# pierotofy/OpenSplat

Hardware: NVIDIA H100
Metric: fwd_bwd_mpixel_per_s (higher is better)
Workload: dtype f32

## Files before the change

### opensplat_b200/csrc/raster_bwd.cu

```cuda
#include "raster_common.cuh"

int gsb_blend_grid(const void *kernel, int num_tiles);

namespace {

__device__ __forceinline__ float rcp_approx(float x) {
    float y;
    asm("rcp.approx.ftz.f32 %0, %1;" : "=f"(y) : "f"(x));
    return y;
}

__device__ __forceinline__ void zero_row(float *grad_rows, int k) {
    float4 *row = reinterpret_cast<float4 *>(grad_rows + (size_t)k * GSB_GRAD_ROW_FLOATS);
    const float4 z = make_float4(0.f, 0.f, 0.f, 0.f);
    row[0] = z; row[1] = z; row[2] = z;
}

constexpr int BWD_MIN_BLOCKS = 6;
template <bool SAT>
__global__ void __launch_bounds__(RK_THREADS, BWD_MIN_BLOCKS)
rasterize_backward_kernel(int img_h, int img_w, int tiles_x, int num_tiles,
                          const int2 *__restrict__ tile_bins, const GsbRecord *__restrict__ records,
                          const float *__restrict__ background, const float *__restrict__ final_Ts,
                          const int *__restrict__ final_idx, const float *__restrict__ v_output,
                          const float *__restrict__ v_output_alpha, float *__restrict__ grad_rows,
                          unsigned *__restrict__ tile_counter, const int *__restrict__ tile_order) {
    __shared__ WarpRing rings[RK_WARPS];
    const int warp = threadIdx.x >> 5, lane = threadIdx.x & 31;
    WarpRing &ring = rings[warp];
    if (lane == 0) {
#pragma unroll
        for (int s = 0; s < RK_STAGES; ++s) mbar_init(&ring.full[s], 1);
        mbar_fence_init();
    }
    __syncwarp();
    const float bg0 = __ldg(background), bg1 = __ldg(background + 1), bg2 = __ldg(background + 2);
    unsigned gchunk = 0;

    while (true) {
        int tile = 0;
        if (lane == 0) tile = (int)atomicAdd(tile_counter, 1u);
        tile = __shfl_sync(0xffffffffu, tile, 0);
        if (tile >= num_tiles) break;
        if (tile_order) tile = __ldg(tile_order + tile);
        const int2 range = tile_bins[tile];
        if (range.y <= range.x) continue;

        const int tx = tile % tiles_x, ty = tile / tiles_x;
        const int X = tx * GSB_TILE + (lane & 15);
        const int Y0 = ty * GSB_TILE + (lane >> 4);
        const float px = (float)X;
        const float tile_x0 = (float)(tx * GSB_TILE), tile_y0 = (float)(ty * GSB_TILE);

        float T[RK_PIX], Bq[RK_PIX];
        const float py0 = (float)Y0;
        float vor[RK_PIX], vog[RK_PIX], vob[RK_PIX];
        int binf[RK_PIX];
        int my_max = -1;
#pragma unroll
        for (int j = 0; j < RK_PIX; ++j) {
            const int Y = Y0 + 2 * j;
            if (X < img_w && Y < img_h) {
                const size_t p = (size_t)Y * img_w + X;
                const float Tf = final_Ts[p];
                T[j] = Tf;
                vor[j] = v_output[3 * p]; vog[j] = v_output[3 * p + 1]; vob[j] = v_output[3 * p + 2];
                binf[j] = final_idx[p];
                if (SAT) {
                    const int f = binf[j];
                    if (f & GSB_SAT_BIT0) vor[j] = 0.f;
                    if (f & (GSB_SAT_BIT0 << 1)) vog[j] = 0.f;
                    if (f & (GSB_SAT_BIT0 << 2)) vob[j] = 0.f;
                    binf[j] = f & ~GSB_SAT_MASK;
                }
                const float voa = v_output_alpha ? v_output_alpha[p] : 0.f;
                Bq[j] = -(Tf * (voa - (bg0 * vor[j] + bg1 * vog[j] + bg2 * vob[j])));
            } else {
                T[j] = 1.f; vor[j] = vog[j] = vob[j] = 0.f; Bq[j] = 0.f;
                binf[j] = -1;
            }
            my_max = max(my_max, binf[j]);
        }
        const int warp_max = __reduce_max_sync(0xffffffffu, my_max);
        const int hi = min(range.y - 1, max(warp_max, range.x - 1));

        for (int idx = hi + 1 + lane; idx < range.y; idx += 32)
            zero_row(grad_rows, __float_as_int(__ldg(&records[idx].q0.w)));
        const int L = hi - range.x + 1;
        if (L <= 0) continue;
        const int nchunks = (L + RK_CHUNK - 1) / RK_CHUNK;

        const unsigned g0 = gchunk;
        auto stage_of = [&](int c) { return (g0 + (unsigned)c) % RK_STAGES; };
        auto parity_of = [&](int c) { return ((g0 + (unsigned)c) / RK_STAGES) & 1u; };
        auto chunk_lo = [&](int c) { return max(range.x, hi + 1 - (c + 1) * RK_CHUNK); };
        auto chunk_cnt = [&](int c) { return (hi + 1 - c * RK_CHUNK) - chunk_lo(c); };
        auto issue = [&](int c) {
            if (lane == 0) {
                const unsigned s = stage_of(c);
                const uint32_t bytes = (uint32_t)chunk_cnt(c) * (uint32_t)sizeof(GsbRecord);
                mbar_arrive_expect_tx(&ring.full[s], bytes);
                tma_load_1d(&ring.rec[s][0], records + chunk_lo(c), bytes, &ring.full[s]);
            }
        };
        const int pro = min(RK_STAGES, nchunks);
        for (int c = 0; c < pro; ++c) issue(c);
        int issued = pro;

        for (int c = 0; c < nchunks; ++c) {
            const unsigned s = stage_of(c);
            mbar_wait(&ring.full[s], parity_of(c));
            const int lo = chunk_lo(c), cnt = chunk_cnt(c);
            unsigned my_mask = 0;
            if (lane < cnt) {
                my_mask = record_slot_mask(ring.rec[s][lane], tile_x0, tile_y0);
                if (my_mask == 0u) zero_row(grad_rows, __float_as_int(ring.rec[s][lane].q0.w));
            }
            unsigned live = __ballot_sync(0xffffffffu, my_mask != 0u);
            while (live) {
                const int t = 31 - __clz(live);
                live &= ~(1u << t);
                const unsigned rm = __shfl_sync(0xffffffffu, my_mask, t);
                const int idx = lo + t;
                const float4 q0 = ring.rec[s][t].q0;
                const float4 q1 = ring.rec[s][t].q1;
                const float4 q2 = ring.rec[s][t].q2;
                const float smax = fmaxf(0.f, fmaf(q0.z, GSB_LN2, GSB_SMAX_BIAS));
                const float dx = q0.x - px;
                const float adx2 = q1.x * dx * dx;
                const float bdx = q1.y * dx;
                const float dy0 = q0.y - py0;
                float s0 = 0.f, s1 = 0.f, s2 = 0.f;
                float a_r = 0.f, a_g = 0.f, a_b = 0.f;
                bool any = false;
                const int jlo = __ffs(rm) - 1, jhi = 31 - __clz(rm);
#define GSB_BWD_SLOT(j)                                                                                   \
    {                                                                                                     \
        const float dy = dy0 - (float)(2 * j);                                                                      \
        const float sigma = fmaf(dy, fmaf(q1.z, dy, bdx), adx2);                                          \
        if (__float_as_uint(sigma) <= __float_as_uint(smax)) {                    \
            const float au = ex2_approx(fmaf(sigma, -GSB_LOG2E, q0.z));           \
            const float alpha = fminf(0.99f, au);                                                         \
            if (idx <= binf[j] && alpha >= (1.f / 255.f)) {                                               \
                any = true;                                                                               \
                const float ra = rcp_approx(1.f - alpha);                                                 \
                T[j] *= ra;                                                                               \
                const float fac = alpha * T[j];                                                           \
                a_r = fmaf(fac, vor[j], a_r);                                                             \
                a_g = fmaf(fac, vog[j], a_g);                                                             \
                a_b = fmaf(fac, vob[j], a_b);                                                             \
                const float d = fmaf(q2.z, vob[j], fmaf(q2.y, vog[j], q2.x * vor[j]));   \
                const float v_alpha = fmaf(d, T[j], -(ra * Bq[j]));                                       \
                Bq[j] = fmaf(d, fac, Bq[j]);                                                              \
                 \
                const float w = au * v_alpha;                                                             \
                const float wdy = w * dy;                                                                 \
                s0 += w;                                                                                  \
                s1 += wdy;                                                                                \
                s2 = fmaf(wdy, dy, s2);                                                                   \
            }                                                                                             \
        }                                                                                                 \
        if (jhi == j) break;                                                                              \
    }
                switch (jlo) {
                    case 0: GSB_BWD_SLOT(0)
                    case 1: GSB_BWD_SLOT(1)
                    case 2: GSB_BWD_SLOT(2)
                    case 3: GSB_BWD_SLOT(3)
                    case 4: GSB_BWD_SLOT(4)
                    case 5: GSB_BWD_SLOT(5)
                    case 6: GSB_BWD_SLOT(6)
                    default: GSB_BWD_SLOT(7)
                }
#undef GSB_BWD_SLOT
                const int k = __float_as_int(q0.w);
                float *row = grad_rows + (size_t)k * GSB_GRAD_ROW_FLOATS;
                if (!__any_sync(0xffffffffu, any)) {
                    if (lane < 9) row[lane] = 0.f;
                    continue;
                }
                const float sx = dx * s0;
                float v0 = s0, v1 = sx, v2 = s1, v3 = dx * sx, v4 = dx * s1, v5 = s2, v6 = a_r, v7 = a_g;
                float v8 = a_b;
                {
                    const bool up = lane & 16;
                    const float t0 = up ? v0 : v4, t1 = up ? v1 : v5, t2 = up ? v2 : v6, t3 = up ? v3 : v7;
                    const float k0 = up ? v4 : v0, k1 = up ? v5 : v1, k2 = up ? v6 : v2, k3 = up ? v7 : v3;
                    v0 = k0 + __shfl_xor_sync(0xffffffffu, t0, 16);
                    v1 = k1 + __shfl_xor_sync(0xffffffffu, t1, 16);
                    v2 = k2 + __shfl_xor_sync(0xffffffffu, t2, 16);
                    v3 = k3 + __shfl_xor_sync(0xffffffffu, t3, 16);
                }
                {
                    const bool up = lane & 8;
                    const float t0 = up ? v0 : v2, t1 = up ? v1 : v3;
                    const float k0 = up ? v2 : v0, k1 = up ? v3 : v1;
                    v0 = k0 + __shfl_xor_sync(0xffffffffu, t0, 8);
                    v1 = k1 + __shfl_xor_sync(0xffffffffu, t1, 8);
                }
                {
                    const bool up = lane & 4;
                    const float t0 = up ? v0 : v1;
                    const float k0 = up ? v1 : v0;
                    v0 = k0 + __shfl_xor_sync(0xffffffffu, t0, 4);
                }
                v0 += __shfl_xor_sync(0xffffffffu, v0, 2);
                v0 += __shfl_xor_sync(0xffffffffu, v0, 1);
#pragma unroll
                for (int o = 16; o > 0; o >>= 1) v8 += __shfl_xor_sync(0xffffffffu, v8, o);
                const bool w8 = (lane == 1);
                if (((lane & 3) == 0) || w8) row[w8 ? 8 : (lane >> 2)] = w8 ? v8 : v0;
            }
            __syncwarp();
            if (issued < nchunks) { issue(issued); ++issued; }
        }
        gchunk = g0 + (unsigned)issued;
        __syncwarp();
    }
}

__global__ void __launch_bounds__(256)
reduce_grad_rows_kernel(int n, const int *__restrict__ cum_tiles_hit, const float *__restrict__ grad_rows,
                        const float *__restrict__ conics, const float *__restrict__ opacities,
                        float2 *__restrict__ v_xy, float *__restrict__ v_conic,
                        float *__restrict__ v_colors, float *__restrict__ v_opacity) {
    const int g = blockIdx.x * blockDim.x + threadIdx.x;
    if (g >= n) return;
    const int k0 = g ? cum_tiles_hit[g - 1] : 0, k1 = cum_tiles_hit[g];
    float a[9] = {0.f, 0.f, 0.f, 0.f, 0.f, 0.f, 0.f, 0.f, 0.f};
    for (int k = k0; k < k1; ++k) {
        const float4 *row = reinterpret_cast<const float4 *>(grad_rows + (size_t)k * GSB_GRAD_ROW_FLOATS);
        const float4 r0 = row[0], r1 = row[1];
        const float r8 = reinterpret_cast<const float *>(row)[8];
        a[0] += r0.x; a[1] += r0.y; a[2] += r0.z; a[3] += r0.w;
        a[4] += r1.x; a[5] += r1.y; a[6] += r1.z; a[7] += r1.w;
        a[8] += r8;
    }
    const float S0 = a[0], Sx = a[1], Sy = a[2], Sxx = a[3], Sxy = a[4], Syy = a[5];
    const float ca = conics[3 * g], cb = conics[3 * g + 1], cc = conics[3 * g + 2];
    const float op = opacities[g];
    v_xy[g] = make_float2(-(ca * Sx + cb * Sy), -(cb * Sx + cc * Sy));
    v_conic[3 * g] = -0.5f * Sxx; v_conic[3 * g + 1] = -0.5f * Sxy; v_conic[3 * g + 2] = -0.5f * Syy;
    v_colors[3 * g] = a[6]; v_colors[3 * g + 1] = a[7]; v_colors[3 * g + 2] = a[8];
    v_opacity[g] = (op > 0.f) ? S0 / op : 0.f;
}

}

extern "C" size_t gsb_raster_grad_rows_bytes(int m) {
    return gsb_align_up((size_t)(m > 0 ? m : 0) * GSB_GRAD_ROW_FLOATS * 4 + 256, 256);
}

extern "C" int gsb_rasterize_backward(int img_h, int img_w, int tiles_x, int tiles_y, int n, int m,
                                      const int32_t *tile_bins, const int32_t *tile_order, const float *conics,
                                      const float *opacities, void *records, const int32_t *cum_tiles_hit,
                                      const float *background, const float *final_Ts, const int32_t *final_idx,
                                      const float *v_output, const float *v_output_alpha, void *grad_rows,
                                      float *v_xy, float *v_conic, float *v_colors, float *v_opacity, unsigned flags,
                                      gsb_stream_t stream) {
    GSB_CHECK_ARG(img_h > 0 && img_w > 0 && n >= 0 && m >= 0);
    GSB_CHECK_ARG((flags & ~(unsigned)GSB_RASTER_CLAMP_MAX_ONE) == 0);
    const bool sat = (flags & GSB_RASTER_CLAMP_MAX_ONE) != 0;
    GSB_CHECK_ARG(tiles_x == gsb_div_up(img_w, GSB_TILE) && tiles_y == gsb_div_up(img_h, GSB_TILE));
    if (n == 0) return 0;
    GSB_CHECK_ARG(tile_bins && conics && opacities && cum_tiles_hit && background && final_Ts && final_idx &&
                  v_output && v_xy && v_conic && v_colors && v_opacity);
    GSB_CHECK_ARG(((uintptr_t)v_xy % 8) == 0);
    cudaStream_t s = (cudaStream_t)stream;
    if (m > 0) {
        GSB_CHECK_ARG(records && grad_rows && ((uintptr_t)records % 16) == 0 && ((uintptr_t)grad_rows % 16) == 0);
        unsigned *counters = reinterpret_cast<unsigned *>(
            reinterpret_cast<char *>(records) + gsb_raster_records_bytes(m) - 256);
        GSB_CUDA(cudaMemsetAsync(counters, 0, 256, s));
        const int num_tiles = tiles_x * tiles_y;
#define GSB_BWD_LAUNCH(S)                                                                                       \
    rasterize_backward_kernel<S><<<gsb_blend_grid((const void *)rasterize_backward_kernel<S>, num_tiles),        \
                                   RK_THREADS, 0, s>>>(                                                         \
        img_h, img_w, tiles_x, num_tiles, reinterpret_cast<const int2 *>(tile_bins),                            \
        reinterpret_cast<const GsbRecord *>(records), background, final_Ts, final_idx, v_output, v_output_alpha, \
        reinterpret_cast<float *>(grad_rows), counters, tile_order)
        if (sat) GSB_BWD_LAUNCH(true); else GSB_BWD_LAUNCH(false);
#undef GSB_BWD_LAUNCH
    }
    reduce_grad_rows_kernel<<<gsb_div_up(n, 256), 256, 0, s>>>(
        n, cum_tiles_hit, reinterpret_cast<const float *>(grad_rows), conics, opacities,
        reinterpret_cast<float2 *>(v_xy), v_conic, v_colors, v_opacity);
    GSB_LAUNCH_CHECK();
    return 0;
}
```

### opensplat_b200/csrc/raster_common.cuh

```cuda
#pragma once
#include "gsb_common.cuh"

struct __align__(16) GsbRecord {
    float4 q0, q1, q2;
};
static_assert(sizeof(GsbRecord) == 48, "record must be 48 bytes");

constexpr int RK_WARPS = 4;
constexpr int RK_THREADS = RK_WARPS * 32;
constexpr int RK_PIX = 8;
constexpr int RK_CHUNK = 32;
constexpr int RK_STAGES = 4;

constexpr float GSB_LN2 = 0.6931471805599453f;
constexpr float GSB_LOG2E = 1.4426950408889634f;
constexpr float GSB_SMAX_BIAS = 5.541263545158426f + 1e-3f;

constexpr int GSB_GRAD_ROW_FLOATS = 12;

constexpr int GSB_SAT_BIT0 = 1 << 28;
constexpr int GSB_SAT_MASK = 7 << 28;

struct __align__(128) WarpRing {
    GsbRecord rec[RK_STAGES][RK_CHUNK];
    uint64_t full[RK_STAGES];
};

#ifdef __CUDACC__
__device__ __forceinline__ GsbRecord make_record(float2 xy, float a, float b, float c, float opac, float r,
                                                 float g, float bl, int k) {
    const float lo = (opac > 0.f) ? log2f(opac) : -INFINITY;
    const float smax = fmaxf(0.f, fmaf(lo, GSB_LN2, GSB_SMAX_BIAS));
    const float det = a * c - b * b;
    float hx = INFINITY, hy = INFINITY;
    if (det > 0.f && a > 0.f && c > 0.f) {
        const float s2 = 2.f * smax / det;
        hx = sqrtf(s2 * c) * 1.001f + 0.01f;
        hy = sqrtf(s2 * a) * 1.001f + 0.01f;
    }
    GsbRecord rec;
    rec.q0 = make_float4(xy.x, xy.y, lo, __int_as_float(k));
    rec.q1 = make_float4(0.5f * a, b, 0.5f * c, hx);
    rec.q2 = make_float4(r, g, bl, hy);
    return rec;
}

__device__ __forceinline__ unsigned extent_slot_mask(float cx, float cy, float hx, float hy, float tile_x0,
                                                     float tile_y0) {
    const float gx = cx - tile_x0, gy = cy - tile_y0;
    const float xlo = fmaxf(ceilf(gx - hx), 0.f), xhi = fminf(floorf(gx + hx), 15.f);
    const float ylo = fmaxf(ceilf(gy - hy), 0.f), yhi = fminf(floorf(gy + hy), 15.f);
    if (!(xlo <= xhi) || !(ylo <= yhi)) return 0u;
    const int jlo = (int)ylo >> 1, jhi = (int)yhi >> 1;
    return ((2u << jhi) - 1u) & ~((1u << jlo) - 1u);
}

__device__ __forceinline__ unsigned record_slot_mask(const GsbRecord &r, float tile_x0, float tile_y0) {
    return extent_slot_mask(r.q0.x, r.q0.y, r.q1.w, r.q2.w, tile_x0, tile_y0);
}
#endif
```

### opensplat_b200/csrc/raster_fwd.cu

```cuda
#include "raster_common.cuh"

namespace {

__global__ void __launch_bounds__(256)
pack_records_kernel(int m, const int *__restrict__ gaussian_ids_sorted,
                    const int *__restrict__ sorted_index, const float2 *__restrict__ xys,
                    const float *__restrict__ conics, const float *__restrict__ colors,
                    const float *__restrict__ opacities, GsbRecord *__restrict__ records) {
    const int i = blockIdx.x * blockDim.x + threadIdx.x;
    if (i >= m) return;
    const int g = gaussian_ids_sorted[i];
    const int k = sorted_index ? sorted_index[i] : i;
    const GsbRecord r = make_record(__ldg(xys + g), __ldg(conics + 3 * g), __ldg(conics + 3 * g + 1),
                                    __ldg(conics + 3 * g + 2), __ldg(opacities + g), __ldg(colors + 3 * g),
                                    __ldg(colors + 3 * g + 1), __ldg(colors + 3 * g + 2), k);
    float4 *dst = reinterpret_cast<float4 *>(records + i);
    stg_stream4(dst, r.q0);
    stg_stream4(dst + 1, r.q1);
    stg_stream4(dst + 2, r.q2);
}

constexpr int FWD_MIN_BLOCKS = 8;
template <bool COUNT, bool SAT>
__global__ void __launch_bounds__(RK_THREADS, FWD_MIN_BLOCKS)
rasterize_forward_kernel(int img_h, int img_w, int tiles_x, int num_tiles,
                         const int2 *__restrict__ tile_bins, const GsbRecord *__restrict__ records,
                         const float *__restrict__ background, float *__restrict__ out_img,
                         float *__restrict__ final_Ts, int *__restrict__ final_idx,
                         unsigned *__restrict__ tile_counter, const int *__restrict__ bin_stats,
                         unsigned long long *__restrict__ pair_counts, const int *__restrict__ tile_order) {
    if (bin_stats && bin_stats[2]) return;
    __shared__ WarpRing rings[RK_WARPS];
    const int warp = threadIdx.x >> 5, lane = threadIdx.x & 31;
    WarpRing &ring = rings[warp];
    if (lane == 0) {
#pragma unroll
        for (int s = 0; s < RK_STAGES; ++s) mbar_init(&ring.full[s], 1);
        mbar_fence_init();
    }
    __syncwarp();
    const float bg0 = __ldg(background), bg1 = __ldg(background + 1), bg2 = __ldg(background + 2);
    unsigned gchunk = 0;
    unsigned long long n_rec = 0, n_slot = 0, n_eval = 0, n_blend = 0;

    while (true) {
        int tile = 0;
        if (lane == 0) tile = (int)atomicAdd(tile_counter, 1u);
        tile = __shfl_sync(0xffffffffu, tile, 0);
        if (tile >= num_tiles) break;
        if (tile_order) tile = __ldg(tile_order + tile);

        const int tx = tile % tiles_x, ty = tile / tiles_x;
        const int X = tx * GSB_TILE + (lane & 15);
        const int Y0 = ty * GSB_TILE + (lane >> 4);
        const float px = (float)X;
        const float tile_x0 = (float)(tx * GSB_TILE), tile_y0 = (float)(ty * GSB_TILE);
        const int2 range = tile_bins[tile];
        const int L = range.y - range.x;
        const int nchunks = (L + RK_CHUNK - 1) / RK_CHUNK;

        float T[RK_PIX], cr[RK_PIX], cg[RK_PIX], cb[RK_PIX];
        const float py0 = (float)Y0;
        int last[RK_PIX];
        unsigned done = 0;
#pragma unroll
        for (int j = 0; j < RK_PIX; ++j) {
            T[j] = 1.f; cr[j] = cg[j] = cb[j] = 0.f; last[j] = 0;
            if (X >= img_w || Y0 + 2 * j >= img_h) { done |= 1u << j; T[j] = -1.f; }
        }

        const unsigned g0 = gchunk;
        auto stage_of = [&](int c) { return (g0 + (unsigned)c) % RK_STAGES; };
        auto parity_of = [&](int c) { return ((g0 + (unsigned)c) / RK_STAGES) & 1u; };
        auto issue = [&](int c) {
            if (lane == 0) {
                const int cnt = min(RK_CHUNK, L - c * RK_CHUNK);
                const uint32_t bytes = (uint32_t)cnt * (uint32_t)sizeof(GsbRecord);
                const unsigned s = stage_of(c);
                mbar_arrive_expect_tx(&ring.full[s], bytes);
                tma_load_1d(&ring.rec[s][0], records + range.x + c * RK_CHUNK, bytes, &ring.full[s]);
            }
        };
        const int pro = min(RK_STAGES, nchunks);
        for (int c = 0; c < pro; ++c) issue(c);
        int issued = pro;

        int c = 0;
        for (; c < nchunks; ++c) {
            const unsigned s = stage_of(c);
            mbar_wait(&ring.full[s], parity_of(c));
            const int cnt = min(RK_CHUNK, L - c * RK_CHUNK);
            const int idx0 = range.x + c * RK_CHUNK;
            unsigned my_mask = 0;
            if (lane < cnt) my_mask = record_slot_mask(ring.rec[s][lane], tile_x0, tile_y0);
            unsigned live = __ballot_sync(0xffffffffu, my_mask != 0u);
            if (COUNT && lane == 0) n_rec += __popc(live);
            while (live) {
                const int t = __ffs(live) - 1;
                live &= live - 1;
                const unsigned rm = __shfl_sync(0xffffffffu, my_mask, t);
                const float4 q0 = ring.rec[s][t].q0;
                const float4 q1 = ring.rec[s][t].q1;
                const float4 q2 = ring.rec[s][t].q2;
                const float smax = fmaxf(0.f, fmaf(q0.z, GSB_LN2, GSB_SMAX_BIAS));
                const float dx = q0.x - px;
                const float adx2 = q1.x * dx * dx;
                const float bdx = q1.y * dx;
                const float dy0 = q0.y - py0;
                const int idx = idx0 + t;
                const int jhi = 31 - __clz(rm);
#define GSB_FWD_SLOT(j)                                                                                   \
    {                                                                                                     \
        const float dy = dy0 - (float)(2 * j);                                                                      \
                                      \
        const float sigma = fmaf(dy, fmaf(q1.z, dy, bdx), adx2);                                          \
        if (COUNT && lane == 0) ++n_slot;                                                                 \
        if (__float_as_uint(sigma) <= __float_as_uint(smax)) {            \
                     \
            const float alpha = fminf(0.999f, ex2_approx(fmaf(sigma, -GSB_LOG2E, q0.z)));                 \
            if (COUNT) ++n_eval;                                                                          \
            if (alpha >= (1.f / 255.f)) {                                                                 \
                const float next_T = T[j] * (1.f - alpha);                                                \
                if (next_T <= 1e-4f) {                                     \
                    if (T[j] > 0.f) { T[j] = -T[j]; done |= 1u << j; }                                    \
                } else {                                                                                  \
                    const float vis = alpha * T[j];                                                       \
                    cr[j] = fmaf(q2.x, vis, cr[j]);                                                       \
                    cg[j] = fmaf(q2.y, vis, cg[j]);                                                       \
                    cb[j] = fmaf(q2.z, vis, cb[j]);                                                       \
                    T[j] = next_T;                                                                        \
                    last[j] = idx;                                                                        \
                    if (COUNT) ++n_blend;                                                                 \
                }                                                                                         \
            }                                                                                             \
        }                                                                                                 \
        if (jhi == j) break;                                                                              \
    }
                do {
                    if (rm & 1u) GSB_FWD_SLOT(0)
                    if (rm & 2u) GSB_FWD_SLOT(1)
                    if (rm & 4u) GSB_FWD_SLOT(2)
                    if (rm & 8u) GSB_FWD_SLOT(3)
                    if (rm & 16u) GSB_FWD_SLOT(4)
                    if (rm & 32u) GSB_FWD_SLOT(5)
                    if (rm & 64u) GSB_FWD_SLOT(6)
                    if (rm & 128u) GSB_FWD_SLOT(7)
                } while (0);
#undef GSB_FWD_SLOT
            }
            if (__all_sync(0xffffffffu, done == 0xffu)) { ++c; break; }
            __syncwarp();
            if (issued < nchunks) { issue(issued); ++issued; }
        }
        for (; c < issued; ++c) mbar_wait(&ring.full[stage_of(c)], parity_of(c));
        gchunk = g0 + (unsigned)issued;
        __syncwarp();

#pragma unroll
        for (int j = 0; j < RK_PIX; ++j) {
            const int Y = Y0 + 2 * j;
            if (X < img_w && Y < img_h) {
                const size_t p = (size_t)Y * img_w + X;
                const float Tf = fabsf(T[j]);
                final_Ts[p] = Tf;
                float o0 = cr[j] + Tf * bg0, o1 = cg[j] + Tf * bg1, o2 = cb[j] + Tf * bg2;
                int fi = last[j];
                if (SAT) {
                    if (!(o0 <= 1.f)) { fi |= GSB_SAT_BIT0; o0 = o0 > 1.f ? 1.f : o0; }
                    if (!(o1 <= 1.f)) { fi |= GSB_SAT_BIT0 << 1; o1 = o1 > 1.f ? 1.f : o1; }
                    if (!(o2 <= 1.f)) { fi |= GSB_SAT_BIT0 << 2; o2 = o2 > 1.f ? 1.f : o2; }
                }
                final_idx[p] = fi;
                out_img[3 * p] = o0;
                out_img[3 * p + 1] = o1;
                out_img[3 * p + 2] = o2;
            }
        }
    }
    if (COUNT) {
        n_eval = __reduce_add_sync(0xffffffffu, (unsigned)n_eval);
        n_blend = __reduce_add_sync(0xffffffffu, (unsigned)n_blend);
        if (lane == 0) {
            atomicAdd(pair_counts + 0, n_rec);
            atomicAdd(pair_counts + 1, n_slot);
            atomicAdd(pair_counts + 2, n_eval);
            atomicAdd(pair_counts + 3, n_blend);
        }
    }
}


}

int gsb_sm_count();
int gsb_blend_grid(const void *kernel, int num_tiles);

extern "C" size_t gsb_raster_records_bytes(int m) {
    return gsb_align_up((size_t)(m > 0 ? m : 0) * sizeof(GsbRecord), 256) + 256;
}

extern "C" int gsb_pack_records(int m, const int32_t *gaussian_ids_sorted, const int32_t *sorted_index,
                                const float *xys, const float *conics, const float *colors, const float *opacities,
                                void *records, gsb_stream_t stream) {
    GSB_CHECK_ARG(m >= 0);
    if (m == 0) return 0;
    GSB_CHECK_ARG(records && gaussian_ids_sorted && xys && conics && colors && opacities);
    GSB_CHECK_ARG(((uintptr_t)records % 16) == 0 && ((uintptr_t)xys % 8) == 0);
    pack_records_kernel<<<gsb_div_up(m, 256), 256, 0, (cudaStream_t)stream>>>(
        m, gaussian_ids_sorted, sorted_index, reinterpret_cast<const float2 *>(xys), conics, colors, opacities,
        reinterpret_cast<GsbRecord *>(records));
    GSB_LAUNCH_CHECK();
    return 0;
}

static int blend_setup(int img_h, int img_w, int tiles_x, int tiles_y, int m, const int32_t *tile_bins,
                       const float *background, void *records, float *out_img, float *final_Ts, int32_t *final_idx,
                       cudaStream_t s, unsigned **counters) {
    GSB_CHECK_ARG(img_h > 0 && img_w > 0 && m >= 0);
    GSB_CHECK_ARG(tiles_x == gsb_div_up(img_w, GSB_TILE) && tiles_y == gsb_div_up(img_h, GSB_TILE));
    GSB_CHECK_ARG(tile_bins && background && out_img && final_Ts && final_idx && records);
    GSB_CHECK_ARG(((uintptr_t)records % 16) == 0);
    *counters = reinterpret_cast<unsigned *>(reinterpret_cast<char *>(records) + gsb_raster_records_bytes(m) - 256);
    GSB_CUDA(cudaMemsetAsync(*counters, 0, 256, s));
    return 0;
}

extern "C" int gsb_rasterize_forward_packed(int img_h, int img_w, int tiles_x, int tiles_y, int m,
                                            const int32_t *tile_bins, const int32_t *tile_order,
                                            const int32_t *bin_stats, const float *background, void *records,
                                            float *out_img, float *final_Ts, int32_t *final_idx, unsigned flags,
                                            gsb_stream_t stream) {
    GSB_CHECK_ARG((flags & ~(unsigned)GSB_RASTER_CLAMP_MAX_ONE) == 0);
    const bool sat = (flags & GSB_RASTER_CLAMP_MAX_ONE) != 0;
    GSB_CHECK_ARG(!sat || m < GSB_SAT_BIT0);
    cudaStream_t s = (cudaStream_t)stream;
    unsigned *counters = nullptr;
    const int rc = blend_setup(img_h, img_w, tiles_x, tiles_y, m, tile_bins, background, records, out_img, final_Ts,
                               final_idx, s, &counters);
    if (rc) return rc;
    const int num_tiles = tiles_x * tiles_y;
#define GSB_FWD_LAUNCH(S)                                                                                        \
    rasterize_forward_kernel<false, S><<<gsb_blend_grid((const void *)rasterize_forward_kernel<false, S>, num_tiles), \
                                         RK_THREADS, 0, s>>>(                                                    \
        img_h, img_w, tiles_x, num_tiles, reinterpret_cast<const int2 *>(tile_bins),                             \
        reinterpret_cast<const GsbRecord *>(records), background, out_img, final_Ts, final_idx, counters,        \
        bin_stats, nullptr, tile_order)
    if (sat) GSB_FWD_LAUNCH(true); else GSB_FWD_LAUNCH(false);
#undef GSB_FWD_LAUNCH
    GSB_LAUNCH_CHECK();
    return 0;
}

extern "C" int gsb_rasterize_forward_count(int img_h, int img_w, int tiles_x, int tiles_y, int m,
                                           const int32_t *tile_bins, const float *background, void *records,
                                           float *out_img, float *final_Ts, int32_t *final_idx,
                                           unsigned long long *pair_counts, gsb_stream_t stream) {
    GSB_CHECK_ARG(pair_counts);
    cudaStream_t s = (cudaStream_t)stream;
    unsigned *counters = nullptr;
    const int rc = blend_setup(img_h, img_w, tiles_x, tiles_y, m, tile_bins, background, records, out_img, final_Ts,
                               final_idx, s, &counters);
    if (rc) return rc;
    const int num_tiles = tiles_x * tiles_y;
    const int grid = gsb_blend_grid((const void *)rasterize_forward_kernel<true, false>, num_tiles);
    rasterize_forward_kernel<true, false><<<grid, RK_THREADS, 0, s>>>(
        img_h, img_w, tiles_x, num_tiles, reinterpret_cast<const int2 *>(tile_bins),
        reinterpret_cast<const GsbRecord *>(records), background, out_img, final_Ts, final_idx, counters, nullptr,
        pair_counts, nullptr);
    GSB_LAUNCH_CHECK();
    return 0;
}

int gsb_sm_count() {
    static thread_local int cached_dev = -1, cached = 0;
    int dev = 0;
    cudaGetDevice(&dev);
    if (dev != cached_dev) {
        cudaDeviceGetAttribute(&cached, cudaDevAttrMultiProcessorCount, dev);
        if (cached <= 0) cached = 132;
        cached_dev = dev;
    }
    return cached;
}

int gsb_blend_grid(const void *kernel, int num_tiles) {
    struct Entry { const void *kernel; int dev; int per_sm; };
    static thread_local Entry cache[8] = {};
    int dev = 0;
    cudaGetDevice(&dev);
    int per_sm = 0;
    for (const Entry &e : cache)
        if (e.kernel == kernel && e.dev == dev) per_sm = e.per_sm;
    if (per_sm == 0) {
        if (cudaOccupancyMaxActiveBlocksPerMultiprocessor(&per_sm, kernel, RK_THREADS, 0) != cudaSuccess || per_sm < 1)
            per_sm = 1;
        for (Entry &e : cache)
            if (e.kernel == nullptr || e.kernel == kernel) { e = Entry{kernel, dev, per_sm}; break; }
    }
    const int full = gsb_sm_count() * per_sm;
    const int need = gsb_div_up(num_tiles, RK_WARPS);
    return need < full ? need : full;
}
```

Before: 1091.

## Move backward per-pixel output grads to shared memory and raise occupancy

After: 1108 (median of 6 runs). 1.5% higher.

```diff
diff --git a/opensplat_b200/csrc/raster_bwd.cu b/opensplat_b200/csrc/raster_bwd.cu
--- a/opensplat_b200/csrc/raster_bwd.cu
+++ b/opensplat_b200/csrc/raster_bwd.cu
@@ -16,7 +16,14 @@
     row[0] = z; row[1] = z; row[2] = z;
 }
 
-constexpr int BWD_MIN_BLOCKS = 6;
+constexpr int BWD_MIN_BLOCKS = 8;
+constexpr int BWD_STAGES = 2;
+
+struct __align__(128) BwdWarpSmem {
+    WarpRing<BWD_STAGES> ring;
+    float v[3][RK_PIX * 32];
+};
+
 template <bool SAT>
 __global__ void __launch_bounds__(RK_THREADS, BWD_MIN_BLOCKS)
 rasterize_backward_kernel(int img_h, int img_w, int tiles_x, int num_tiles,
@@ -25,12 +32,13 @@
                           const int *__restrict__ final_idx, const float *__restrict__ v_output,
                           const float *__restrict__ v_output_alpha, float *__restrict__ grad_rows,
                           unsigned *__restrict__ tile_counter, const int *__restrict__ tile_order) {
-    __shared__ WarpRing rings[RK_WARPS];
+    __shared__ BwdWarpSmem smem[RK_WARPS];
     const int warp = threadIdx.x >> 5, lane = threadIdx.x & 31;
-    WarpRing &ring = rings[warp];
+    WarpRing<BWD_STAGES> &ring = smem[warp].ring;
+    float (*const vo)[RK_PIX * 32] = smem[warp].v;
     if (lane == 0) {
 #pragma unroll
-        for (int s = 0; s < RK_STAGES; ++s) mbar_init(&ring.full[s], 1);
+        for (int s = 0; s < BWD_STAGES; ++s) mbar_init(&ring.full[s], 1);
         mbar_fence_init();
     }
     __syncwarp();
@@ -54,31 +62,32 @@
 
         float T[RK_PIX], Bq[RK_PIX];
         const float py0 = (float)Y0;
-        float vor[RK_PIX], vog[RK_PIX], vob[RK_PIX];
         int binf[RK_PIX];
         int my_max = -1;
 #pragma unroll
         for (int j = 0; j < RK_PIX; ++j) {
             const int Y = Y0 + 2 * j;
+            float vor = 0.f, vog = 0.f, vob = 0.f;
             if (X < img_w && Y < img_h) {
                 const size_t p = (size_t)Y * img_w + X;
                 const float Tf = final_Ts[p];
                 T[j] = Tf;
-                vor[j] = v_output[3 * p]; vog[j] = v_output[3 * p + 1]; vob[j] = v_output[3 * p + 2];
+                vor = v_output[3 * p]; vog = v_output[3 * p + 1]; vob = v_output[3 * p + 2];
                 binf[j] = final_idx[p];
                 if (SAT) {
                     const int f = binf[j];
-                    if (f & GSB_SAT_BIT0) vor[j] = 0.f;
-                    if (f & (GSB_SAT_BIT0 << 1)) vog[j] = 0.f;
-                    if (f & (GSB_SAT_BIT0 << 2)) vob[j] = 0.f;
+                    if (f & GSB_SAT_BIT0) vor = 0.f;
+                    if (f & (GSB_SAT_BIT0 << 1)) vog = 0.f;
+                    if (f & (GSB_SAT_BIT0 << 2)) vob = 0.f;
                     binf[j] = f & ~GSB_SAT_MASK;
                 }
                 const float voa = v_output_alpha ? v_output_alpha[p] : 0.f;
-                Bq[j] = -(Tf * (voa - (bg0 * vor[j] + bg1 * vog[j] + bg2 * vob[j])));
+                Bq[j] = -(Tf * (voa - (bg0 * vor + bg1 * vog + bg2 * vob)));
             } else {
-                T[j] = 1.f; vor[j] = vog[j] = vob[j] = 0.f; Bq[j] = 0.f;
+                T[j] = 1.f; Bq[j] = 0.f;
                 binf[j] = -1;
             }
+            vo[0][32 * j + lane] = vor; vo[1][32 * j + lane] = vog; vo[2][32 * j + lane] = vob;
             my_max = max(my_max, binf[j]);
         }
         const int warp_max = __reduce_max_sync(0xffffffffu, my_max);
@@ -91,8 +100,8 @@
         const int nchunks = (L + RK_CHUNK - 1) / RK_CHUNK;
 
         const unsigned g0 = gchunk;
-        auto stage_of = [&](int c) { return (g0 + (unsigned)c) % RK_STAGES; };
-        auto parity_of = [&](int c) { return ((g0 + (unsigned)c) / RK_STAGES) & 1u; };
+        auto stage_of = [&](int c) { return (g0 + (unsigned)c) % BWD_STAGES; };
+        auto parity_of = [&](int c) { return ((g0 + (unsigned)c) / BWD_STAGES) & 1u; };
         auto chunk_lo = [&](int c) { return max(range.x, hi + 1 - (c + 1) * RK_CHUNK); };
         auto chunk_cnt = [&](int c) { return (hi + 1 - c * RK_CHUNK) - chunk_lo(c); };
         auto issue = [&](int c) {
@@ -103,7 +112,7 @@
                 tma_load_1d(&ring.rec[s][0], records + chunk_lo(c), bytes, &ring.full[s]);
             }
         };
-        const int pro = min(RK_STAGES, nchunks);
+        const int pro = min(BWD_STAGES, nchunks);
         for (int c = 0; c < pro; ++c) issue(c);
         int issued = pro;
 
@@ -146,10 +155,12 @@
                 const float ra = rcp_approx(1.f - alpha);                                                 \
                 T[j] *= ra;                                                                               \
                 const float fac = alpha * T[j];                                                           \
-                a_r = fmaf(fac, vor[j], a_r);                                                             \
-                a_g = fmaf(fac, vog[j], a_g);                                                             \
-                a_b = fmaf(fac, vob[j], a_b);                                                             \
-                const float d = fmaf(q2.z, vob[j], fmaf(q2.y, vog[j], q2.x * vor[j]));   \
+                const float vor = vo[0][32 * j + lane], vog = vo[1][32 * j + lane];                       \
+                const float vob = vo[2][32 * j + lane];                                                   \
+                a_r = fmaf(fac, vor, a_r);                                                                \
+                a_g = fmaf(fac, vog, a_g);                                                                \
+                a_b = fmaf(fac, vob, a_b);                                                                \
+                const float d = fmaf(q2.z, vob, fmaf(q2.y, vog, q2.x * vor));            \
                 const float v_alpha = fmaf(d, T[j], -(ra * Bq[j]));                                       \
                 Bq[j] = fmaf(d, fac, Bq[j]);                                                              \
                  \
diff --git a/opensplat_b200/csrc/raster_common.cuh b/opensplat_b200/csrc/raster_common.cuh
--- a/opensplat_b200/csrc/raster_common.cuh
+++ b/opensplat_b200/csrc/raster_common.cuh
@@ -10,7 +10,6 @@
 constexpr int RK_THREADS = RK_WARPS * 32;
 constexpr int RK_PIX = 8;
 constexpr int RK_CHUNK = 32;
-constexpr int RK_STAGES = 4;
 
 constexpr float GSB_LN2 = 0.6931471805599453f;
 constexpr float GSB_LOG2E = 1.4426950408889634f;
@@ -21,9 +20,10 @@
 constexpr int GSB_SAT_BIT0 = 1 << 28;
 constexpr int GSB_SAT_MASK = 7 << 28;
 
+template <int STAGES>
 struct __align__(128) WarpRing {
-    GsbRecord rec[RK_STAGES][RK_CHUNK];
-    uint64_t full[RK_STAGES];
+    GsbRecord rec[STAGES][RK_CHUNK];
+    uint64_t full[STAGES];
 };
 
 #ifdef __CUDACC__
diff --git a/opensplat_b200/csrc/raster_fwd.cu b/opensplat_b200/csrc/raster_fwd.cu
--- a/opensplat_b200/csrc/raster_fwd.cu
+++ b/opensplat_b200/csrc/raster_fwd.cu
@@ -21,6 +21,7 @@
 }
 
 constexpr int FWD_MIN_BLOCKS = 8;
+constexpr int FWD_STAGES = 4;
 template <bool COUNT, bool SAT>
 __global__ void __launch_bounds__(RK_THREADS, FWD_MIN_BLOCKS)
 rasterize_forward_kernel(int img_h, int img_w, int tiles_x, int num_tiles,
@@ -30,12 +31,12 @@
                          unsigned *__restrict__ tile_counter, const int *__restrict__ bin_stats,
                          unsigned long long *__restrict__ pair_counts, const int *__restrict__ tile_order) {
     if (bin_stats && bin_stats[2]) return;
-    __shared__ WarpRing rings[RK_WARPS];
+    __shared__ WarpRing<FWD_STAGES> rings[RK_WARPS];
     const int warp = threadIdx.x >> 5, lane = threadIdx.x & 31;
-    WarpRing &ring = rings[warp];
+    WarpRing<FWD_STAGES> &ring = rings[warp];
     if (lane == 0) {
 #pragma unroll
-        for (int s = 0; s < RK_STAGES; ++s) mbar_init(&ring.full[s], 1);
+        for (int s = 0; s < FWD_STAGES; ++s) mbar_init(&ring.full[s], 1);
         mbar_fence_init();
     }
     __syncwarp();
@@ -70,8 +71,8 @@
         }
 
         const unsigned g0 = gchunk;
-        auto stage_of = [&](int c) { return (g0 + (unsigned)c) % RK_STAGES; };
-        auto parity_of = [&](int c) { return ((g0 + (unsigned)c) / RK_STAGES) & 1u; };
+        auto stage_of = [&](int c) { return (g0 + (unsigned)c) % FWD_STAGES; };
+        auto parity_of = [&](int c) { return ((g0 + (unsigned)c) / FWD_STAGES) & 1u; };
         auto issue = [&](int c) {
             if (lane == 0) {
                 const int cnt = min(RK_CHUNK, L - c * RK_CHUNK);
@@ -81,7 +82,7 @@
                 tma_load_1d(&ring.rec[s][0], records + range.x + c * RK_CHUNK, bytes, &ring.full[s]);
             }
         };
-        const int pro = min(RK_STAGES, nchunks);
+        const int pro = min(FWD_STAGES, nchunks);
         for (int c = 0; c < pro; ++c) issue(c);
         int issued = pro;
 
```
